# IbrahimSquared/visibility-heuristic-path-planner

Measured on AMD Instinct MI355X. Metric: visibility fields/sec on 1000x1000 grid, higher is better.
Workload: dtype f64

## Files before the change

visibility-heuristic-path-planner_amd/csrc/vhp_diag.h:

```cpp
#pragma once

#ifdef VHP_DIAG_NOSTORE
#define VHP_DIAG_STORE_GUARD(a, b, off) { asm volatile("" :: "v"(a), "v"(b), "v"(off)); return; }
#define VHP_DIAG_FRONT_STORE_GUARD if (nx != 0x7fffffff) return;
#else
#define VHP_DIAG_STORE_GUARD(a, b, off)
#define VHP_DIAG_FRONT_STORE_GUARD
#endif

#ifdef VHP_DIAG_NOXSTORE
#define VHP_DIAG_NOXSTORE_RETURN return;
#else
#define VHP_DIAG_NOXSTORE_RETURN
#endif
#ifdef VHP_DIAG_NOYSTORE
#define VHP_DIAG_NOYSTORE_RETURN return;
#define VHP_DIAG_NOYSTORE_GUARD if (m.nx == 0x7fffffff)
#else
#define VHP_DIAG_NOYSTORE_RETURN
#define VHP_DIAG_NOYSTORE_GUARD
#endif

#ifdef VHP_DIAG_PLAINSTORE
#define VHP_FIELD_STORE_PLAIN 1
#endif

#ifdef VHP_DIAG_NOWAIT
#define VHP_DIAG_NOWAIT_RETURN return;
#define VHP_DIAG_WAITS false
#else
#define VHP_DIAG_NOWAIT_RETURN
#define VHP_DIAG_WAITS true
#endif

#ifdef VHP_DIAG_NOMATH
#define VHP_DIAG_NOMATH_RETURN(x) return (x);
#else
#define VHP_DIAG_NOMATH_RETURN(x)
#endif

#if defined(VHP_DIAG_TIMELINE) && !defined(VHP_SIM)
#define VHP_DIAG_TL_DECLARE                                                                                                     \
  constexpr int kPpBins = 256;                                                                                                  \
  static __device__ unsigned long long g_pp_hist[256 * 2 * kPpBins];                                                            \
  static __device__ unsigned long long g_pp_t0;                                                                                 \
  static __device__ unsigned g_pp_unit[16384 * 2];    \
  static __device__ __forceinline__ unsigned long long* pp_slot(int which) {                                                    \
    const unsigned long long b_ = (wall_clock64() - g_pp_t0) / 1000;                                                            \
    return g_pp_hist + ((size_t)(blockIdx.x & 255) * 2 + which) * kPpBins + (b_ < kPpBins - 1 ? b_ : kPpBins - 1);              \
  }
#define VHP_DIAG_TL_ADD(which, n) do { if ((threadIdx.x & 63) == 0) atomicAdd(pp_slot(which), (unsigned long long)(long long)(n)); } while (0)
#define VHP_DIAG_TL_STRIPS(d) VHP_DIAG_TL_ADD(1, d);
#define VHP_DIAG_TL_UNIT(unit, which) do { if ((threadIdx.x & 63) == 0 && (unit) < 16384) g_pp_unit[2 * (unit) + (which)] = (unsigned)(wall_clock64() - g_pp_t0); } while (0);
#define VHP_DIAG_TL_XBLOCK(lo, hi, rows_here, j0, cb) { long c_ = 0; for (int i_ = (lo); i_ <= (hi); ++i_) c_ += ((rows_here) < i_ - (j0) + 1 ? (rows_here) : i_ - (j0) + 1); VHP_DIAG_TL_ADD(0, c_ * (cb)); }
#define VHP_DIAG_TL_YBLOCK(lo, hi, i0, ycols, ni, cb) { long c_ = 0; for (int j_ = (lo); j_ <= (hi); ++j_) { int t_ = (i0) + (ycols) - 1; if ((ni) - 1 < t_) t_ = (ni) - 1; if (j_ < t_) t_ = j_; t_ -= ((i0) > 0 ? (i0) : 0) - 1; if (t_ > 0) c_ += t_; } VHP_DIAG_TL_ADD(0, c_ * (cb)); }
#define VHP_DIAG_TL_RESET for (int k_ = threadIdx.x; k_ < 256 * 2 * kPpBins; k_ += blockDim.x) g_pp_hist[k_] = 0; if (threadIdx.x == 0) g_pp_t0 = wall_clock64();
#else
#define VHP_DIAG_TL_DECLARE
#define VHP_DIAG_TL_STRIPS(d)
#define VHP_DIAG_TL_UNIT(unit, which)
#define VHP_DIAG_TL_XBLOCK(lo, hi, rows_here, j0, cb)
#define VHP_DIAG_TL_YBLOCK(lo, hi, i0, ycols, ni, cb)
#define VHP_DIAG_TL_RESET
#endif

#ifndef VHP_PRIO_DIAG
#define VHP_PRIO_DIAG 1
#endif
#ifndef VHP_PRIO_TASK
#define VHP_PRIO_TASK 2
#endif
#if !defined(VHP_SIM) && defined(VHP_PRIO_MARCH)
#define VHP_EXP_PRIO_SET_LEFT(is_diag, left) wave_priority((is_diag) ? 3 : (left) >= VHP_PRIO_MARCH ? 2 : (left) >= VHP_PRIO_MARCH / 2 ? 1 : 0);
#define VHP_EXP_PRIO_SET(is_diag) wave_priority((is_diag) ? 3 : 0);
#define VHP_EXP_PRIO_TASK_BEGIN wave_priority(3);
#define VHP_EXP_PRIO_END wave_priority(0);
#elif !defined(VHP_SIM) && (VHP_PRIO_DIAG != 0 || VHP_PRIO_TASK != 0)
#define VHP_EXP_PRIO_SET_LEFT(is_diag, left) wave_priority((is_diag) ? VHP_PRIO_DIAG : 0);
#define VHP_EXP_PRIO_SET(is_diag) wave_priority((is_diag) ? VHP_PRIO_DIAG : 0);
#define VHP_EXP_PRIO_TASK_BEGIN wave_priority(VHP_PRIO_TASK);
#define VHP_EXP_PRIO_END wave_priority(0);
#else
#define VHP_EXP_PRIO_SET_LEFT(is_diag, left)
#define VHP_EXP_PRIO_SET(is_diag)
#define VHP_EXP_PRIO_TASK_BEGIN
#define VHP_EXP_PRIO_END
#endif

#ifndef VHP_BACKOFF_SLEEP
#define VHP_BACKOFF_SLEEP 12
#endif
#ifndef VHP_READY_SLEEP
#define VHP_READY_SLEEP 4
#endif
```

visibility-heuristic-path-planner_amd/csrc/vhp_pool.hip:

```cpp
#include "vhp_batch_launch.h"

#include <hip/hip_runtime.h>

#include "vhp.h"
#include "vhp_pool.hpp"
#include "vhp_pool_scratch.hpp"

namespace vhp {
namespace pool {

__device__ __forceinline__ void write_stamp(stamps::Entry* p, unsigned long long tag) {
  *reinterpret_cast<ulonglong2*>(p) = make_ulonglong2((unsigned long long)wall_clock64(), tag);
}

template <typename OutT, bool ANYW>
__global__ void __launch_bounds__(64 * kWaves, 1) vhp_pool_sweep(Args<OutT> a, int n_ctx, stamps::Entry* __restrict__ stamp_end) {
  extern __shared__ double lds[];
  constexpr int W = ANYW ? kWavesAny : kWaves;
  const Layout L = make_layout(W, n_ctx, a.m.nx, a.m.ny, ANYW ? kTStrideAny : kTStride);
  Worker<OutT, ANYW>::clear(lds, L, (int)threadIdx.x, 64 * W);
  __syncthreads();
  Worker<OutT, ANYW> wk;
  wk.init(a, lds, L, uniform((int)(threadIdx.x >> 6)), (int)blockIdx.x);
  wk.run();
  if (stamp_end) {
    asm volatile("s_waitcnt vmcnt(0)" ::: "memory");
    __syncthreads();
    if (threadIdx.x == 0) write_stamp(stamp_end + blockIdx.x, a.epoch);
  }
}

constexpr int kOrderLdsUnits = 8192;

template <typename Arr>
__device__ __forceinline__ int block_exclusive_scan_1024(Arr arr, int n, int* wave_tot) {
  const int per = (n + 1023) / 1024;
  const int lo = (int)threadIdx.x * per, hi = lo + per < n ? lo + per : n;
  int mine = 0;
  for (int k = lo; k < hi; ++k) mine += arr[k];
  const int lane = threadIdx.x & 63, wv = threadIdx.x >> 6;
  int inc = mine;
#pragma unroll
  for (int off = 1; off < 64; off <<= 1) {
    const int t = __shfl_up(inc, off, 64);
    if (lane >= off) inc += t;
  }
  if (lane == 63) wave_tot[wv] = inc;
  __syncthreads();
  int before = 0, all = 0;
#pragma unroll
  for (int k = 0; k < 16; ++k) { before += k < wv ? wave_tot[k] : 0; all += wave_tot[k]; }
  int at = before + inc - mine;
  for (int k = lo; k < hi; ++k) { const int v = arr[k]; arr[k] = at; at += v; }
  __syncthreads();
  return all;
}

template <typename PerUnit>
__device__ __forceinline__ void order_units(const int32_t* __restrict__ src_xy, int n_src, int nx, int ny, int* __restrict__ order,
                                            int* __restrict__ line_base, int* __restrict__ recs, long long capacity_blocks,
                                            unsigned long long* __restrict__ queue, unsigned long long queue0,
                                            int* __restrict__ err_flag, int* hist, int* wave_tot, PerUnit blocks) {
  const int n_units = n_src * kUnits;
  const double inv_area = 1.0 / ((double)nx * (double)ny), inv_side = 1.0 / (double)(nx > ny ? nx : ny);
  hist[threadIdx.x] = 0;
  __syncthreads();
  for (int u = threadIdx.x; u < n_units; u += 1024) {
    const int s = u / kUnits, qo = u - s * kUnits;
    const int sx = src_xy[2 * s], sy = src_xy[2 * s + 1];
    int nb = 0, bucket = kBuckets - 1;
    if (!(sx < 0 || sy < 0 || sx >= nx || sy >= ny)) {
      UnitGeo g;
      g.init(nx, ny, qo, sx, sy);
      nb = g.line_blocks();
      bucket = unit_launch_bucket(g, inv_area, inv_side);
    }
    blocks[u] = nb | (bucket << 20);
    atomicAdd(&hist[bucket], 1);
  }
  __syncthreads();
  (void)block_exclusive_scan_1024(hist, kBuckets, wave_tot);
  for (int u = threadIdx.x; u < n_units; u += 1024) order[atomicAdd(&hist[blocks[u] >> 20], 1)] = u;
  __syncthreads();
  for (int u = threadIdx.x; u < n_units; u += 1024) blocks[u] &= (1 << 20) - 1;
  __syncthreads();
  const int total = block_exclusive_scan_1024(blocks, n_units, wave_tot);
  const bool fits = (long long)total <= capacity_blocks;
  for (int k = threadIdx.x; k < n_units; k += 1024) {
    const int u = order[k], s = u / kUnits;
    const int sx = src_xy[2 * s], sy = src_xy[2 * s + 1];
    const bool inside = !(sx < 0 || sy < 0 || sx >= nx || sy >= ny);
    reinterpret_cast<int4*>(recs)[k] = make_int4(u, !fits ? -2 : inside ? (sx | (sy << 16)) : -1, blocks[u], 0);
  }
  if (threadIdx.x == 0) {
    *queue = fits ? queue0 : (unsigned long long)n_units;
    if (!fits) atomicOr(err_flag, 4);
  }
}

__device__ __forceinline__ void order_units_lds(const int32_t* __restrict__ src_xy, int n_src, int nx, int ny, int* __restrict__ recs,
                                                long long capacity_blocks, unsigned long long* __restrict__ queue, unsigned long long queue0,
                                                int* __restrict__ err_flag, int* hist, int* wave_tot, int* unit_key, int* src_key) {
  const int n_units = n_src * kUnits;
  const int per = (n_units + 1023) / 1024;
  const int lo = (int)threadIdx.x * per, hi = lo + per < n_units ? lo + per : n_units;
  const double inv_area = 1.0 / ((double)nx * (double)ny), inv_side = 1.0 / (double)(nx > ny ? nx : ny);
  hist[threadIdx.x] = 0;
  __syncthreads();
  int mine = 0;
  for (int u = lo; u < hi; ++u) {
    const int s = u / kUnits, qo = u - s * kUnits;
    const int sx = src_xy[2 * s], sy = src_xy[2 * s + 1];
    const bool inside = !(sx < 0 || sy < 0 || sx >= nx || sy >= ny);
    int nb = 0, bucket = kBuckets - 1;
    if (inside) {
      UnitGeo g;
      g.init(nx, ny, qo, sx, sy);
      nb = g.line_blocks();
      bucket = unit_launch_bucket(g, inv_area, inv_side);
    }
    unit_key[u] = nb | (bucket << 20);
    if (qo == 0) src_key[s] = inside ? (sx | (sy << 16)) : -1;
    mine += nb;
    atomicAdd(&hist[bucket], 1);
  }
  __syncthreads();
  const int lane = threadIdx.x & 63, wv = threadIdx.x >> 6;
  const int count = hist[threadIdx.x];
  int inc_h = count, inc_b = mine;
#pragma unroll
  for (int off = 1; off < 64; off <<= 1) {
    const int th = __shfl_up(inc_h, off, 64), tb = __shfl_up(inc_b, off, 64);
    if (lane >= off) { inc_h += th; inc_b += tb; }
  }
  if (lane == 63) { wave_tot[wv] = inc_h; wave_tot[16 + wv] = inc_b; }
  __syncthreads();
  int before_h = 0, before_b = 0, total = 0;
#pragma unroll
  for (int k = 0; k < 16; ++k) {
    before_h += k < wv ? wave_tot[k] : 0;
    before_b += k < wv ? wave_tot[16 + k] : 0;
    total += wave_tot[16 + k];
  }
  hist[threadIdx.x] = before_h + inc_h - count;
  __syncthreads();
  const bool fits = (long long)total <= capacity_blocks;
  int at = before_b + inc_b - mine;
  for (int u = lo; u < hi; ++u) {
    const int key = unit_key[u], nb = key & ((1 << 20) - 1);
    const int k = atomicAdd(&hist[key >> 20], 1);
    reinterpret_cast<int4*>(recs)[k] = make_int4(u, !fits ? -2 : src_key[u / kUnits], at, 0);
    at += nb;
  }
  if (threadIdx.x == 0) {
    *queue = fits ? queue0 : (unsigned long long)n_units;
    if (!fits) atomicOr(err_flag, 4);
  }
}

__global__ void __launch_bounds__(1024) vhp_pool_order(const int32_t* __restrict__ src_xy, int n_src, int nx, int ny, int* __restrict__ order,
                                                       int* __restrict__ line_base, int* __restrict__ recs, long long capacity_blocks,
                                                       unsigned long long* __restrict__ queue, unsigned long long queue0,
                                                       int* __restrict__ err_flag, stamps::Entry* __restrict__ stamp_begin,
                                                       unsigned long long stamp_tag) {
  if (stamp_begin && threadIdx.x == 0) write_stamp(stamp_begin, stamp_tag);
  __shared__ int hist[kBuckets];
  __shared__ int wave_tot[32];
  __shared__ int blocks[kOrderLdsUnits];
  __shared__ int src_key[kOrderLdsUnits / kUnits];
  VHP_DIAG_TL_RESET
  if (n_src * kUnits <= kOrderLdsUnits) order_units_lds(src_xy, n_src, nx, ny, recs, capacity_blocks, queue, queue0, err_flag, hist, wave_tot, blocks, src_key);
  else order_units(src_xy, n_src, nx, ny, order, line_base, recs, capacity_blocks, queue, queue0, err_flag, hist, wave_tot, line_base);
}

}

namespace {
template <typename OutT>
hipError_t launch_pool_t(const BatchArgs& a) {
  using namespace pool;
  const bool anyw = pool_needs_anyw<OutT>(a.nx, a.field_stride > 0 ? a.field_stride : (long long)a.nx * a.ny, static_cast<const OutT*>(a.d_out));
  auto k = anyw ? vhp_pool_sweep<OutT, true> : vhp_pool_sweep<OutT, false>;
  const PoolPlan p = plan_pool(a.nx, a.ny, a.n_src, a.n_cus, anyw, a.pool);
  if (!p.ok || a.pool_epoch == 0) return hipErrorInvalidValue;
  if (a.raise_lds) {
    hipError_t e = a.raise_lds(reinterpret_cast<const void*>(k), p.lds_bytes);
    if (e != hipSuccess) return e;
  }
  char* scratch = reinterpret_cast<char*>(a.d_queue);
  Args<OutT> g;
  g.m = geom_map(a);
  g.out = static_cast<OutT*>(a.d_out);
  g.field_stride = a.field_stride;
  g.err_flag = a.d_err;
  g.queue = reinterpret_cast<unsigned long long*>(a.d_queue);
  g.n_units = a.n_src * kUnits;
  int* recs = a.d_queue + kQueueInts;
  int* order = recs + 4 * (size_t)g.n_units;
  int* line_base = order + g.n_units;
  g.recs = recs;
  g.diag = reinterpret_cast<double*>(scratch + head_bytes(a.n_src));
  g.diag_stride = diag_stride_of(a.nx, a.ny);
  g.lines = reinterpret_cast<vhp::lanes::Tagged*>(scratch + head_bytes(a.n_src) + diag_bytes(a.n_src, a.nx, a.ny));
  g.epoch = a.pool_epoch;
  g.busy_cap = p.busy_cap;
  g.n_head = p.n_head;
  g.tail_limit = p.tail_limit;
  g.early_ctx = p.early_ctx;
  g.late_after = p.late_after;
  g.claim_ahead = p.claim_ahead;
  g.n_groups = a.n_cus;
  g.static_snake = p.static_snake;
  g.static_round = p.static_round;
  stamps::Entry* const stamp_end = a.d_stamps ? a.d_stamps + pool_stamp_counts(a.n_cus).n_begin : nullptr;
  if (a.ev_begin) (void)hipEventRecord(a.ev_begin, a.stream);
  hipLaunchKernelGGL(vhp_pool_order, dim3(1), dim3(1024), 0, a.stream, a.d_src, a.n_src, a.nx, a.ny, order, line_base, recs,
                     line_blocks_per_source(a.nx, a.ny) * a.n_src, reinterpret_cast<unsigned long long*>(a.d_queue), p.queue0, a.d_err,
                     a.d_stamps, a.pool_epoch);
  hipLaunchKernelGGL(k, dim3((unsigned)a.n_cus), dim3(64 * p.waves), p.lds_bytes, a.stream, g, p.n_ctx, stamp_end);
  const hipError_t e = hipGetLastError();
  if (a.ev_end) (void)hipEventRecord(a.ev_end, a.stream);
  return e;
}
}

size_t pool_scratch_bytes(int n_src, int nx, int ny) {
  return head_bytes(n_src) + diag_bytes(n_src, nx, ny) + (size_t)line_blocks_per_source(nx, ny) * (size_t)n_src * 64 * sizeof(vhp::lanes::Tagged);
}

#ifdef VHP_DIAG_TIMELINE
extern "C" int vhp_debug_read_hist(unsigned long long* dst, int n_words) {
  return (int)hipMemcpyFromSymbol(dst, HIP_SYMBOL(pool::g_pp_hist), (size_t)n_words * 8);
}
extern "C" int vhp_debug_read_units(unsigned* dst, int n_words) {
  return (int)hipMemcpyFromSymbol(dst, HIP_SYMBOL(pool::g_pp_unit), (size_t)n_words * 4);
}
#endif

hipError_t launch_pool(const BatchArgs& a) {
  if (!pool_supported(a.nx, a.ny)) return hipErrorInvalidValue;
  return a.dtype == VHP_F64 ? launch_pool_t<double>(a) : launch_pool_t<float>(a);
}

}
```

visibility-heuristic-path-planner_amd/csrc/vhp_pool.hpp:

```cpp
#pragma once
#include "vhp_geom.hpp"

namespace vhp {
namespace pool {

using namespace vhp::lanes;
using geom::imax;
using geom::imin;
using geom::Map;
using geom::Quad;

constexpr int kBlock = geom::kBlock;
constexpr int kXRows = geom::kXRows;
constexpr int kYCols = geom::kYCols;
constexpr int kLW16 = 16;
constexpr int kTStride = 17;
constexpr int kTStrideAny = 25;
constexpr int kUnits = 8;
VHP_DIAG_TL_DECLARE

constexpr int kSchedHead = 8 + 16, kCtxHead = 8;
constexpr int kHdr = 8;
constexpr int kBin = 72;
constexpr int kRing = 256;
// ... 905 lines not shown
        const vi mp = DX > 0 ? lane : 63 - lane;
        const vb end = (mp < head) || (mp >= tail);
        g_store2_mask(!end, row - 2, xoff + (uint32_t)(3 * CB), hi, nb);
        g_store2_if(end && oknb, end && !oknb, vb(false), row - 2, xoff + (uint32_t)(3 * CB), hi, nb);
      } else
        g_store2_if(okhi && oknb, okhi, oknb, row - 2, xoff + (uint32_t)(3 * CB), hi, nb);
      g_store1_if((lane == (DX > 0 ? 0 : 63)) && oklo, row, xoff, lo);
      return;
    }
    if (PRED) g_store2_if(oklo && okhi, oklo, okhi, row, xoff, lo, hi);
    else if (ANYW && VHP_POOL_SPLIT_ENDS) {
      const uint32_t k = (static_cast<uint32_t>(reinterpret_cast<uintptr_t>(row)) + static_cast<uint32_t>(piece_lo * CB)) & 63u;
      if (k == 0) { g_store2(row, xoff, lo, hi); return; }
      const int head = (int)((64u - k) / (2 * CB)), tail = 64 - (int)(k / (2 * CB));
      const vi ml = DX > 0 ? lane : 63 - lane;
      const vb end = (ml < head) || (ml >= tail);
      g_store2_mask(!end, row, xoff, lo, hi);
      g_store2_if(end, vb(false), vb(false), row, xoff, lo, hi);
    }
    else g_store2(row, xoff, lo, hi);
  }
  VHP_FN bool row_aligned(const OutT* row) const { return (reinterpret_cast<uintptr_t>(row) & (2 * CB - 1)) == 0; }
  VHP_FN OutT* row_ptr(int y) const { return out + (size_t)y * (size_t)m.nx; }

  VHP_FN void step1(int j) {
    const int y = g.Y(j);
    const int t = y & 63;
    const double rj = slab[t];
    const double dj = (double)j;
    double fill = 0.0;
    if (q > 0) fill = bin[1 + (y & 63) - DY];
    const vd b0 = shift_up(prev1, vd(fill));
    vd v0 = and_mask(stencil(prev0, b0, ratio(id0, dj, rj)), bit_mask(ow0, t));
    vd v1 = and_mask(stencil(prev1, prev0, ratio(id1, dj, rj)), bit_mask(ow1, t));
    if (j <= i0 + kYCols - 1) {
      v0 = select(ia == j, dg0, v0);
      v1 = select(ib == j, dg1, v1);
    }
    store_row<true>(row_ptr(y), j, v0, v1);
    prev0 = v0;
    prev1 = v1;
    if (has_consumer) lds_store_if(lane == 63, lk.ring, vi(y & (kRing - 1)), v1);
  }

  template <bool DIAG, bool PRED>
  VHP_FN void window8(int j0w) {
    const int y0 = g.Y(j0w);
    const int t0 = y0 & 63;
    const int yb = y0 & ~7;
    vd rr[8];
#pragma unroll
    for (int k = 0; k < 8; ++k) rr[k] = lds_bcast(slab, (yb & 63) + (DY > 0 ? k : 7 - k));
    vd rb[8];
#pragma unroll
    for (int k = 0; k < 8; ++k) rb[k] = vd(0.0);
    if (q > 0) {
      rb[0] = lds_bcast(bin, 1 + (y0 & 63) - DY);
      const int yq = 1 + (yb & 63);
#pragma unroll
      for (int k = 1; k < 8; ++k) rb[k] = lds_bcast(bin, yq + (DY > 0 ? k - 1 : 8 - k));
    }
    const int sh = DY > 0 ? (t0 & 31) : (t0 & 31) - 7;
    const vu32 hs0 = half_shifted(ow0, t0, sh), hs1 = half_shifted(ow1, t0, sh);
    double* wbase = has_consumer ? lk.ring + (yb & (kRing - 1)) : dummy;
    const vi widx = select(lane == 63, vi(0), vi((int)(dummy - wbase)));
    vd dj = vd((double)j0w);
    OutT* row = row_ptr(y0);
    const long rowstep = (long)DY * m.nx;
#pragma unroll
    for (int k = 0; k < 8; ++k) {
      const int bit = DY > 0 ? k : 7 - k;
      const vd b0 = shift_up(prev1, rb[k]);
      vd v0 = and_mask(stencil(prev0, b0, ratio(id0, dj, rr[k])), sbfe1(hs0, bit));
      vd v1 = and_mask(stencil(prev1, prev0, ratio(id1, dj, rr[k])), sbfe1(hs1, bit));
      if (DIAG) {
        v0 = select(ia == j0w + k, dg0, v0);
        v1 = select(ib == j0w + k, dg1, v1);
      }
      store_row<PRED>(row, j0w + k, v0, v1);
      prev0 = v0;
      prev1 = v1;
      lds_store(wbase, widx + bit, v1);
      dj = dj + 1.0;
      row += rowstep;
    }
  }

  VHP_FN void sweep_block(int nb) {
    int lo, hi;
    g.ysteps(nb, lo, hi);
    lo = imax(lo, jstart);
    if (lo > hi) return;
    VHP_EXP_PRIO_SET(lo <= i0 + kYCols - 1)
    const int blk = g.Y(lo) >> 6;
    {
      const vi xa = vmin(vmax(ia, 0), g.ni - 1) * DX + g.sx;
      const vi xb = vmin(vmax(ib, 0), g.ni - 1) * DX + g.sx;
      ow0 = g_load_u64(m.cols, xa * m.wpc + (1 + blk));
      ow1 = g_load_u64(m.cols, xb * m.wpc + (1 + blk));
      const vi jt = (lane + (blk * 64 - g.sy)) * DY;
      const vb ok = (jt >= 0) && (jt < g.nj);
      vd rv = select(ok, g_load_f64(m.recip, select(ok, jt, vi(0))), vd(0.0));
      pin(ow0);
      pin(ow1);
      pin(rv);
      lds_store(slab, lane, rv);
      wave_sync();
    }
    int j = lo;
    while (j <= hi) {
      const int y = g.Y(j);
      const bool aligned = DY > 0 ? (y & 7) == 0 : (y & 7) == 7;
      if (aligned && j + 7 <= hi) {
        if (q > 0) lk.fetch(j, j + 7, nb);
        if (j <= i0 + kYCols - 1) window8<true, true>(j);
        else if (!interior) window8<false, true>(j);
        else window8<false, false>(j);
        j += 8;
      } else {
        if (q > 0) lk.fetch(j, j, nb);
        step1(j);
        j += 1;
      }
      if (has_consumer) lk.publish(j);
    }
    if (has_consumer) lk.store_block(nb, blk);
    VHP_DIAG_TL_YBLOCK(lo, hi, i0, kYCols, g.ni, CB)
  }
};

template <int DX, int DY, typename OutT>
struct YStrip16 {
  static constexpr int CB = sizeof(OutT);
  static constexpr int kW = 16;
  static constexpr int kNever = 0x7fffffff;
  Map m;
  Quad<DX, DY> g;
  OutT* out;
  double* slab;
  double* bin;
  double* dummy;
  Link<DY> lk;
  int q, i0, j_first, j_last;
  bool below, has_consumer, interior;
  int blk, pf_blk, staged_blk;
  bool pf_wait;
  int tl_lo;
  vi lane, ia, ib;
  vi f0, f1;
  vd prev0, prev1, id0, id1, dg0, dg1;
  vu64 ow0, ow1, ow0_nx, ow1_nx;
  vd rv_nx;
  vu32 xoff;

  VHP_FN void init(const Map& m_, int sx, int sy, OutT* out_, const Shared& sh, int w, int q_, const double* diag) {
    m = m_; out = out_;
    g.init(m.nx, m.ny, sx, sy);
    slab = sh.lds + sh.L.slabs + w * (2 * kBlock);
    bin = lk.bin;
    dummy = sh.lds + sh.L.dummies + w * 8;
    lane = lane_id();
    q = q_;
    i0 = g.ycol0(q);
    j_first = g.ystart(q);
    j_last = g.nj - 1;
    below = q > 0;
    has_consumer = q + 1 < g.Py;
    interior = i0 >= 0 && i0 + kYCols - 1 < g.ni;
    ia = lane * 2 + i0;
    ib = ia + 1;
    prev0 = vd(0.0);
    prev1 = vd(0.0);
    id0 = to_f64(ia);
    id1 = to_f64(ib);
    const vb real0 = (ia >= 0) && (ia < g.ni), real1 = (ib >= 0) && (ib < g.ni);
    const vb zero1 = (DX < 0) ? ((ib == g.ni) && real0) : vb(false);
    f0 = select(real0, ia, vi(kNever));
    f1 = select(real1, ib, select(zero1, ia, vi(kNever)));
    dg0 = g_load_f64(diag, vmin(vmax(ia, 0), g.rows_total - 1));
    dg1 = g_load_f64(diag, vmin(vmax(ib, 0), g.rows_total - 1));
    pin(dg0);
    pin(dg1);
    dg1 = select(zero1, vd(0.0), dg1);
    const vi xlo = DX > 0 ? ia + g.sx : (-ib) + g.sx;
    xoff = to_u32(xlo * CB);
    pf_blk = -1;
    pf_wait = false;
    staged_blk = -0x7fffffff;
    blk = -0x7fffffff;
    tl_lo = j_first;
  }

  VHP_FN void load_ops(int b, vu64& o0, vu64& o1, vd& rv) {
    const vi xa = vmin(vmax(ia, 0), g.ni - 1) * DX + g.sx;
    const vi xb = vmin(vmax(ib, 0), g.ni - 1) * DX + g.sx;
    o0 = g_load_u64(m.cols, xa * m.wpc + (1 + b));
    o1 = g_load_u64(m.cols, xb * m.wpc + (1 + b));
    if (DX < 0) o1 = select(ib == g.ni, vu64(0), o1);
    const vi jt = (lane + (b * 64 - g.sy)) * DY;
    const vb ok = (jt >= 0) && (jt < g.nj);
    rv = select(ok, g_load_f64(m.recip, select(ok, jt, vi(0))), vd(0.0));
  }
  VHP_FN bool block_in_march(int b) const { const int ye = g.Y(j_last); return DY > 0 ? 64 * b <= ye : 64 * b + 63 >= ye; }
  VHP_FN void prefetch_ops(int b) { pf_blk = b; pf_wait = true; load_ops(b, ow0_nx, ow1_nx, rv_nx); }
  VHP_FN void stage(int b, vd rv) {
    wave_sync();
    lds_store(slab, lane + kBlock * (b & 1), rv);
    wave_sync();
    staged_blk = b;
  }
  VHP_FN void settle() {
    if (pf_wait) { pin(ow0_nx); pin(ow1_nx); pin(rv_nx); pf_wait = false; }
  }
  VHP_FN void stage_next() {
    if (pf_blk != -1 && staged_blk != pf_blk) { settle(); stage(pf_blk, rv_nx); }
  }
  VHP_FN void enter_block(int b) {
    if (pf_blk == b) { stage_next(); ow0 = ow0_nx; ow1 = ow1_nx; }
    else { vd rv; load_ops(b, ow0, ow1, rv); pin(ow0); pin(ow1); pin(rv); stage(b, rv); }
    blk = b;
    if (block_in_march(b + DY)) prefetch_ops(b + DY); else pf_blk = -1;
  }

  template <bool DIAG, bool PRED>
  VHP_FN void window(int ja, int yw, int nb) {
    const int k_hi = imin(kW - 1, j_last - ja);
    vd rr[kW];
#pragma unroll
    for (int k = 0; k < kW; ++k) rr[k] = lds_bcast(slab, (yw & (2 * kBlock - 1)) + (DY > 0 ? k : kW - 1 - k));
    Below16<DY> bl;
    if (below) bl.get(lk, bin, yw, DY > 0 ? yw : yw + kW - 1, imax(ja, j_first), ja + k_hi - 1, nb);
    const vu32 hs0 = half_shifted(ow0, yw & 63, yw & 31), hs1 = half_shifted(ow1, yw & 63, yw & 31);
    double* wbase = has_consumer ? lk.ring + (yw & (kRing - 1)) : dummy;
    const vi widx = select(lane == 63, vi(0), vi((int)(dummy - wbase)));
    vd dj = vd((double)ja);
    OutT* row = out + (long)g.Y(ja) * (long)m.nx;
    const long rowstep = (long)DY * m.nx;
#pragma unroll
    for (int k = 0; k < kW; ++k) {
      const int c = DY > 0 ? k : kW - 1 - k;
      const vd b0 = shift_up(prev1, below ? bl.v[k] : vd(0.0));
      vd v0 = and_mask(stencil(prev0, b0, ratio(id0, dj, rr[k])), sbfe1(hs0, c));
      vd v1 = and_mask(stencil(prev1, prev0, ratio(id1, dj, rr[k])), sbfe1(hs1, c));
      if (DIAG) {
        v0 = select(ia == ja + k, dg0, v0);
        v1 = select(ib == ja + k, dg1, v1);
      }
      VHP_DIAG_NOYSTORE_GUARD
      {
        const vd lo = DX > 0 ? v0 : v1, hi = DX > 0 ? v1 : v0;
        if (PRED) {
          const int j = ja + k <= j_last ? ja + k : -1;
          const vb ok0 = f0 <= j, ok1 = f1 <= j;
          const vb oklo = DX > 0 ? ok0 : ok1, okhi = DX > 0 ? ok1 : ok0;
          g_store2_if(oklo && okhi, oklo, okhi, row, xoff, lo, hi);
        } else {
          g_store2(row, xoff, lo, hi);
        }
      }
      prev0 = v0;
      prev1 = v1;
      lds_store(wbase, widx + c, v1);
      dj = dj + 1.0;
      row += rowstep;
    }
    if (has_consumer) lk.publish(ja + k_hi + 1);
  }

  VHP_FN void open_block(int yw, int ja) {
    const int b = yw >> 6;
    if (b == blk) return;
    if (has_consumer) lk.store_block(g.nby(ja - 1), blk);
    VHP_DIAG_TL_YBLOCK(tl_lo, ja - 1, i0, kYCols, g.ni, CB)
    tl_lo = ja;
    VHP_EXP_PRIO_SET_LEFT(ja <= i0 + kYCols - 1, j_last - ja)
    enter_block(b);
  }
  VHP_FN void run() {
    int yw = g.Y(j_first) & ~(kW - 1);
    int ja = DY > 0 ? yw - g.sy : g.sy - (yw + kW - 1);
    VHP_EXP_PRIO_SET(true)
    enter_block(yw >> 6);
    while (ja <= j_last) {
      open_block(yw, ja);
      const int nb = DY > 0 ? blk - g.by0 : g.by0 - blk;
      if (ja <= i0 + kYCols - 1) window<true, true>(ja, yw, nb);
      else if (!interior || ja + kW - 1 > j_last) window<false, true>(ja, yw, nb);
      else window<false, false>(ja, yw, nb);
      ja += kW; yw += kW * DY;
      sim_progress();
      sim_point();
    }
    if (has_consumer) lk.store_block(imax(g.nby(imin(imax(ja - 1, 0), j_last)), 0), blk);
    VHP_DIAG_TL_YBLOCK(tl_lo, j_last, i0, kYCols, g.ni, CB)
  }
};

template <int DX, int DY>
struct DiagTask {
  Map m;
  Quad<DX, DY> g;
  double* diag;
  int k;
  vi lane;
  vd dprev, sprev;

  VHP_FN void init(const Map& m_, int sx, int sy, double* diag_) {
    m = m_;
    g.init(m.nx, m.ny, sx, sy);
    diag = diag_;
    lane = lane_id();
    k = 0;
    dprev = vd(0.0);
    sprev = vd(0.0);
  }
  VHP_FN bool done() const { return k >= g.rows_total; }
  VHP_FN int run_chunk() {
    const int k0 = k, k1 = imin(k0 + kBlock, g.rows_total);
    const vi kk = vmin(lane + k0, g.rows_total - 1);
    const vi x = kk * DX + g.sx;
    const vi ya = vmax(kk - 1, 0) * DY + g.sy, yb = kk * DY + g.sy;
    const vu64 wa = g_load_u64(m.rows, ya * m.wpr + ((x >> 6) + 1));
    const vu64 wb = g_load_u64(m.rows, yb * m.wpr + ((x >> 6) + 1));
    const vd rk = g_load_f64(m.recip, kk);
    const vi ma = bit_mask_lane(wa, x & 63), mb = bit_mask_lane(wb, x & 63);
    const vd cv = ratio(to_f64(vmax(kk - 1, 0)), to_f64(kk), rk);
    vd acc = vd(0.0);
    for (int kq = k0; kq < k1; ++kq) {
      const int l = kq - k0;
      vd dcur;
      if (kq == 0) {
        dcur = and_mask(vd(1.0), vi(read_lane_i(mb, l)));
        sprev = vd(0.0);
      } else {
        const vd c = vd(read_lane(cv, l));
        const vd sub = and_mask(stencil(dprev, sprev, c), vi(read_lane_i(ma, l)));
        dcur = and_mask(sub, vi(read_lane_i(mb, l)));
        sprev = sub;
      }
      dprev = dcur;
      acc = select(lane == l, dcur, acc);
    }
    g_store_f64_if(lane < (k1 - k0), diag, lane + k0, acc);
    k = k1;
    return k1;
  }
};

enum { kFound = 0, kRetry = 1, kIdle = 2, kExit = 3 };


template <typename OutT>
VHP_HD bool pool_needs_anyw(int nx, long long field_stride, const OutT* out) {
  return (nx & 7) != 0 || (field_stride & 1) != 0 || (reinterpret_cast<uintptr_t>(out) & (2 * sizeof(OutT) - 1)) != 0;
}

#ifndef VHP_POOL_X8
#define VHP_POOL_X16 1
#else
#define VHP_POOL_X16 0
#endif

template <typename OutT, bool ANYW = false>
struct Worker {
  static constexpr bool kUseX16 = !ANYW && VHP_POOL_X16 != 0;
#ifdef VHP_POOL_Y8
  static constexpr bool kUseY16 = false, kMayY16 = false;
#else
  static constexpr bool kUseY16 = kUseX16;
#ifdef VHP_POOL_ANYW_Y16
  static constexpr bool kMayY16 = ANYW && VHP_POOL_X16 != 0;
#else
  static constexpr bool kMayY16 = false;
#endif
#endif
  Args<OutT> a;
  Shared sh;
  int w, group;
  bool pairs_aligned;
  vi lane;

  VHP_FN void init(const Args<OutT>& a_, double* lds, const Layout& L, int w_, int group_) {
    a = a_;
    pairs_aligned = (a_.m.nx & 1) == 0 && (a_.field_stride & 1) == 0 && (reinterpret_cast<uintptr_t>(a_.out) & (2 * sizeof(OutT) - 1)) == 0;
    sh.lds = lds;
    sh.L = L;
    w = w_;
    group = group_;
    lane = lane_id();
  }

  static VHP_FN void clear(double* lds, const Layout& L, int tid, int nthreads) {
    Shared s;
    s.lds = lds;
    s.L = L;
    int* sc = s.sched();
    const int n = kSchedHead + L.C * L.ctx_stride;
    for (int k = tid; k < n; k += nthreads) lds_set_int(sc + k, 0);
  }

  VHP_FN int find_work(int& c_out, int& p_out, int& qo_out, int& sx_out, int& sy_out) {
    int* sc = sh.sched();
    int best_c = -1, best_seq = 0x7fffffff, best_p = 0, best_word = 0, best_qo = 0, best_sx = 0, best_sy = 0;
    int free_c = -1, free_first = -1;
    bool unclaimed = false, installing = false;
    const bool late_open = a.early_ctx >= sh.L.C || lds_poll(sc + kLateOpen) != 0;
    const int first_done = a.static_round ? lds_poll(sc + kFirstDone) : -1;
    for (int c = 0; c < sh.L.C; ++c) {
      int* cx = sh.ctx(c);
      const int st = lds_poll(cx + kState);
      if (st == 0) {
        if (((first_done >> c) & 1) == 0) free_first = c;
        else if (c < a.early_ctx || late_open) free_c = c;
        continue;
      }
      if (st == 1) { installing = true; continue; }
      const int word = lds_poll(cx + kWord);
      if (word < 0) continue;
      const int p = word & 255, seq = word >> 8;
      const int ns = lds_poll(cx + kNStrips);
      if (p >= ns) continue;
      unclaimed = true;
      const int rank = c < a.n_head ? c : seq + 16;
      if (rank >= best_seq) continue;
      const int unit = lds_poll(cx + kUnit), sxsy = lds_poll(cx + kSxSy);
      const int qo = unit & 7, sx = sxsy & 0xffff, sy = sxsy >> 16;
      UnitGeo ug;
      ug.init(a.m.nx, a.m.ny, qo, sx, sy);
      if (VHP_DIAG_WAITS && p > 0 && lds_poll(sh.prog(c) + (p - 1)) < ug.first_step(p) + 8 + 1 - a.claim_ahead) continue;
      if (VHP_DIAG_WAITS && !ug.x_major && lds_poll(cx + kDiagReady) < ug.diag_need(p)) continue;
      best_c = c; best_seq = rank; best_p = p; best_word = word; best_qo = qo; best_sx = sx; best_sy = sy;
    }
    if (best_c >= 0) {
      sim_point();
      if (lds_cas(sh.ctx(best_c) + kWord, best_word, best_word + 1) != best_word) return kRetry;
      lds_set_int(sh.owner(best_c) + best_p, w);
      c_out = best_c; p_out = best_p; qo_out = best_qo; sx_out = best_sx; sy_out = best_sy;
      sim_progress();
      return kFound;
    }
    const bool q_empty = lds_poll(sc + kQEmpty) != 0;
    if (free_first >= 0) free_c = free_first;
    if (free_c >= 0 && (!q_empty || free_first >= 0) && lds_poll(sc + kBusy) < a.busy_cap) {
      sim_point();
      if (lds_cas(sh.ctx(free_c) + kState, 0, 1) == 0) {
        install(free_c);
      }
      return kRetry;
    }
    if (q_empty && !unclaimed && !installing && free_first < 0) return kExit;
    return kIdle;
  }

  VHP_FN void install(int c) {
    int* sc = sh.sched();
    int* cx = sh.ctx(c);
    int idx;
    if (a.static_round && ((lds_poll(sc + kFirstDone) >> c) & 1) == 0) {
      lds_or(sc + kFirstDone, 1 << c);
      const int slot = (a.static_snake && (c & 1)) ? a.n_groups - 1 - group : group;
      idx = c < a.n_head ? c * a.n_groups + slot : a.n_units - 1 - ((c - a.n_head) * a.n_groups + group);
      sim_progress();
    } else {
      bool from_tail = c >= a.n_head;
      if (from_tail && (int)(g_peek_u64(a.queue) >> 32) >= a.tail_limit) from_tail = false;
      const unsigned long long old = g_add_u64(a.queue, from_tail ? (1ull << 32) : 1ull);
      const unsigned taken_head = (unsigned)old, taken_tail = (unsigned)(old >> 32);
      idx = from_tail ? a.n_units - 1 - (int)taken_tail : (int)taken_head;
      if ((int)(taken_head + taken_tail) >= a.late_after) lds_publish(sc + kLateOpen, 1);
      sim_progress();
      if (taken_head + taken_tail >= (unsigned)a.n_units) {
        lds_publish(sc + kQEmpty, 1);
        lds_publish(cx + kState, 0);
        return;
      }
    }
    int unit, sxsy, lbase, rsvd;
    g_load_rec4(a.recs, idx, unit, sxsy, lbase, rsvd);
    const int s = unit / kUnits, qo = unit - s * kUnits;
    if (sxsy < 0) {
      if (qo == 0 && sxsy == -1) g_store_scalar_if(lane == 0, a.err_flag, vi(0), 1);
      lds_publish(cx + kState, 0);
      return;
    }
    const int sx = sxsy & 0xffff, sy = sxsy >> 16;
    VHP_DIAG_TL_UNIT(unit, 0)
    UnitGeo ug;
    ug.init(a.m.nx, a.m.ny, qo, sx, sy);
    OutT* field = a.out + (size_t)s * a.field_stride;
    if (qo == 0) {
      if (sy > 0)
        for (int x0 = 0; x0 < a.m.nx; x0 += kLanes) g_store_scalar_if(lane + x0 < a.m.nx, field, lane + x0, OutT(0));
    }
    if (ug.n_strips == 0) {
      lds_publish(cx + kState, 0);
      return;
    }
    lds_set_int(cx + kUnit, unit);
    lds_set_int(cx + kNStrips, ug.n_strips);
    lds_set_int(cx + kLeft, ug.n_strips);
    lds_set_int(cx + kSxSy, sxsy);
    lds_set_int(cx + kDiagReady, 0);
    lds_set_int(cx + kLineBase, lbase);
    for (int k0 = 0; k0 < ug.n_strips; k0 += kLanes) lds_store_i_if(lane + k0 < ug.n_strips, sh.prog(c), lane + k0, 0);
    const int seq = lds_add(sc + kSeq, 1) + 1;
    lds_publish(cx + kWord, seq << 8);
    lds_publish(cx + kState, 2);
    if (!ug.x_major) {
      double* dline = a.diag + (size_t)(4 * s + (qo >> 1)) * a.diag_stride;
      switch (qo >> 1) {
        case 0: run_diag<+1, +1>(cx, sx, sy, dline); break;
        case 1: run_diag<-1, +1>(cx, sx, sy, dline); break;
        case 2: run_diag<-1, -1>(cx, sx, sy, dline); break;
        default: run_diag<+1, -1>(cx, sx, sy, dline); break;
      }
    }
  }

  template <int DX, int DY>
  VHP_FN void run_diag(int* cx, int sx, int sy, double* dline) {
    DiagTask<DX, DY> dt;
    dt.init(a.m, sx, sy, dline);
    VHP_EXP_PRIO_TASK_BEGIN
    while (!dt.done()) {
      const int ready = dt.run_chunk();
      stores_done();
      lds_publish(cx + kDiagReady, ready);
      sim_progress();
      sim_point();
    }
    VHP_EXP_PRIO_END
  }

  VHP_FN void strip_done(int c) {
    int* cx = sh.ctx(c);
    if (lds_add(cx + kLeft, -1) == 1) {
      VHP_DIAG_TL_UNIT(lds_int_at(cx + kUnit), 1)
      lds_publish(cx + kWord, -1);
      lds_publish(cx + kState, 0);
    }
    sim_progress();
  }

  VHP_FN Tagged* line_of(int c, int p, int nb) const { return a.lines + (size_t)64 * ((size_t)lds_int_at(sh.ctx(c) + kLineBase) + (size_t)p * nb); }
  VHP_FN int tag_of(int c, int p) const { return (((lds_int_at(sh.ctx(c) + kWord) >> 8) & 0x1ff) << 8) | p; }

  template <int DX, int DY>
  VHP_FN void run_x(int c, int unit, int p, int sx, int sy, OutT* field) {
    Quad<DX, DY> g;
    g.init(a.m.nx, a.m.ny, sx, sy);
    int* mine = sh.prog(c) + p;
    if (kUseX16) {
      XStrip16<DX, DY, OutT> xs;
      xs.lk.init(sh, w, sx, kXRows * p, tag_of(c, p), mine, p > 0 ? line_of(c, p - 1, g.Nbx) : nullptr, p + 1 < g.Px ? line_of(c, p, g.Nbx) : nullptr,
                 a.epoch, p > 0 ? lds_int_at(sh.owner(c) + (p - 1)) : -1, p > 0 ? tag_of(c, p - 1) : 0);
      xs.init(a.m, sx, sy, field, sh, w, p);
      VHP_DIAG_TL_STRIPS(1)
      xs.run();
    } else {
      XStrip<DX, DY, OutT, ANYW> xs;
      xs.lk.init(sh, w, sx, kXRows * p, tag_of(c, p), mine, p > 0 ? line_of(c, p - 1, g.Nbx) : nullptr, p + 1 < g.Px ? line_of(c, p, g.Nbx) : nullptr,
                 a.epoch, p > 0 ? lds_int_at(sh.owner(c) + (p - 1)) : -1, p > 0 ? tag_of(c, p - 1) : 0);
      xs.init(a.m, sx, sy, field, sh, w, p);
      VHP_DIAG_TL_STRIPS(1)
      for (int n = p; n < xs.g.Nbx; ++n) {
        xs.sweep_block(n);
        if (n == xs.g.Nbx - 1) xs.end_of_march();
        sim_progress();
        sim_point();
      }
    }
    lds_publish(mine, 0x3fff);
    VHP_DIAG_TL_STRIPS(-1)
    strip_done(c);
  }

  template <int DX, int DY>
  VHP_FN void run_y(int c, int unit, int q, int sx, int sy, OutT* field, const double* dline) {
    Quad<DX, DY> g;
    g.init(a.m.nx, a.m.ny, sx, sy);
    int* mine = sh.prog(c) + q;
    if (kUseY16 || (kMayY16 && pairs_aligned)) {
      YStrip16<DX, DY, OutT> ys;
      ys.lk.init(sh, w, sy, g.ystart(q), tag_of(c, q), mine, q > 0 ? line_of(c, q - 1, g.Nby) : nullptr, q + 1 < g.Py ? line_of(c, q, g.Nby) : nullptr,
                 a.epoch, q > 0 ? lds_int_at(sh.owner(c) + (q - 1)) : -1, q > 0 ? tag_of(c, q - 1) : 0);
      ys.init(a.m, sx, sy, field, sh, w, q, dline);
      VHP_DIAG_TL_STRIPS(1)
      ys.run();
    } else {
      YStrip<DX, DY, OutT, ANYW> ys;
      ys.lk.init(sh, w, sy, g.ystart(q), tag_of(c, q), mine, q > 0 ? line_of(c, q - 1, g.Nby) : nullptr, q + 1 < g.Py ? line_of(c, q, g.Nby) : nullptr,
                 a.epoch, q > 0 ? lds_int_at(sh.owner(c) + (q - 1)) : -1, q > 0 ? tag_of(c, q - 1) : 0);
      ys.init(a.m, sx, sy, field, sh, w, q, dline);
      VHP_DIAG_TL_STRIPS(1)
      for (int n = ys.g.nby(ys.jstart); n < ys.g.Nby; ++n) {
        ys.sweep_block(n);
        sim_progress();
        sim_point();
      }
    }
    lds_publish(mine, 0x3fff);
    VHP_DIAG_TL_STRIPS(-1)
    strip_done(c);
  }

  VHP_FN void run_strip(int c, int p, int qo, int sx, int sy) {
    const int unit = lds_int_at(sh.ctx(c) + kUnit);
    const int s = unit / kUnits;
    OutT* field = a.out + (size_t)s * a.field_stride;
    const double* dline = a.diag + (size_t)(4 * s + (qo >> 1)) * a.diag_stride;
    switch (qo) {
      case 0: run_x<+1, +1>(c, unit, p, sx, sy, field); break;
      case 1: run_y<+1, +1>(c, unit, p, sx, sy, field, dline); break;
      case 2: run_x<-1, +1>(c, unit, p, sx, sy, field); break;
      case 3: run_y<-1, +1>(c, unit, p, sx, sy, field, dline); break;
      case 4: run_x<-1, -1>(c, unit, p, sx, sy, field); break;
      case 5: run_y<-1, -1>(c, unit, p, sx, sy, field, dline); break;
      case 6: run_x<+1, -1>(c, unit, p, sx, sy, field); break;
      default: run_y<+1, -1>(c, unit, p, sx, sy, field, dline); break;
    }
  }

  VHP_FN void run() {
    for (;;) {
      int c = 0, p = 0, qo = 0, sx = 0, sy = 0;
      const int r = find_work(c, p, qo, sx, sy);
      if (r == kExit) break;
      if (r == kIdle) { backoff(); continue; }
      if (r == kRetry) continue;
      lds_add(sh.sched() + kBusy, 1);
      run_strip(c, p, qo, sx, sy);
      VHP_EXP_PRIO_END
      lds_add(sh.sched() + kBusy, -1);
    }
  }
};

}
}
```

Before: 447,700.

## Limit diagonal precompute to rows consumed by y-strips and add hold-time probes

The diagonal task now stops after the number of entries the y-strips actually consume (kYCols*Py - ya) rather than all rows_total, which drops diagonal work that no strip reads. The diff also adds timeline diagnostics that measure how long y-major strips wait on diagonal readiness, plus per-unit start and diag-done stamps. These diagnostics compile to nothing unless VHP_DIAG_TIMELINE is defined. The risk is a mismatch in the entry count if some consumer needs rows beyond that bound.

```diff
diff --git a/visibility-heuristic-path-planner_amd/csrc/vhp_diag.h b/visibility-heuristic-path-planner_amd/csrc/vhp_diag.h
--- a/visibility-heuristic-path-planner_amd/csrc/vhp_diag.h
+++ b/visibility-heuristic-path-planner_amd/csrc/vhp_diag.h
@@ -44,23 +44,38 @@
   constexpr int kPpBins = 256;                                                                                                  \
   static __device__ unsigned long long g_pp_hist[256 * 2 * kPpBins];                                                            \
   static __device__ unsigned long long g_pp_t0;                                                                                 \
-  static __device__ unsigned g_pp_unit[16384 * 2];    \
+   \
+  static __device__ unsigned g_pp_unit[16384 * 4];                                                                              \
+   \
+  static __device__ unsigned long long g_pp_held[256 * 4];                                                                      \
+  static __device__ unsigned long long g_pp_since[256 * 16];    \
   static __device__ __forceinline__ unsigned long long* pp_slot(int which) {                                                    \
     const unsigned long long b_ = (wall_clock64() - g_pp_t0) / 1000;                                                            \
     return g_pp_hist + ((size_t)(blockIdx.x & 255) * 2 + which) * kPpBins + (b_ < kPpBins - 1 ? b_ : kPpBins - 1);              \
+  }                                                                                                                             \
+  static __device__ __forceinline__ void pp_held(unsigned long long since) {                                                    \
+    if ((threadIdx.x & 63) != 0 || since == 0) return;                                                                          \
+    atomicAdd(g_pp_held + (blockIdx.x & 255) * 4 + 1, 1ull);                                                                    \
+    atomicAdd(g_pp_held + (blockIdx.x & 255) * 4 + 2, wall_clock64() - since);                                                  \
   }
 #define VHP_DIAG_TL_ADD(which, n) do { if ((threadIdx.x & 63) == 0) atomicAdd(pp_slot(which), (unsigned long long)(long long)(n)); } while (0)
 #define VHP_DIAG_TL_STRIPS(d) VHP_DIAG_TL_ADD(1, d);
-#define VHP_DIAG_TL_UNIT(unit, which) do { if ((threadIdx.x & 63) == 0 && (unit) < 16384) g_pp_unit[2 * (unit) + (which)] = (unsigned)(wall_clock64() - g_pp_t0); } while (0);
+#define VHP_DIAG_TL_UNIT(unit, which) do { if ((threadIdx.x & 63) == 0 && (unit) < 16384) g_pp_unit[4 * (unit) + (which)] = (unsigned)(wall_clock64() - g_pp_t0); } while (0);
 #define VHP_DIAG_TL_XBLOCK(lo, hi, rows_here, j0, cb) { long c_ = 0; for (int i_ = (lo); i_ <= (hi); ++i_) c_ += ((rows_here) < i_ - (j0) + 1 ? (rows_here) : i_ - (j0) + 1); VHP_DIAG_TL_ADD(0, c_ * (cb)); }
 #define VHP_DIAG_TL_YBLOCK(lo, hi, i0, ycols, ni, cb) { long c_ = 0; for (int j_ = (lo); j_ <= (hi); ++j_) { int t_ = (i0) + (ycols) - 1; if ((ni) - 1 < t_) t_ = (ni) - 1; if (j_ < t_) t_ = j_; t_ -= ((i0) > 0 ? (i0) : 0) - 1; if (t_ > 0) c_ += t_; } VHP_DIAG_TL_ADD(0, c_ * (cb)); }
-#define VHP_DIAG_TL_RESET for (int k_ = threadIdx.x; k_ < 256 * 2 * kPpBins; k_ += blockDim.x) g_pp_hist[k_] = 0; if (threadIdx.x == 0) g_pp_t0 = wall_clock64();
+#define VHP_DIAG_TL_HELD_MARK(c) do { unsigned long long* s_ = g_pp_since + (blockIdx.x & 255) * 16 + ((c) & 15); if ((threadIdx.x & 63) == 0 && *s_ == 0) *s_ = wall_clock64(); } while (0);
+#define VHP_DIAG_TL_HELD_CLAIM(c, y_major) do { unsigned long long* s_ = g_pp_since + (blockIdx.x & 255) * 16 + ((c) & 15); if (y_major) pp_held(*s_); if ((threadIdx.x & 63) == 0) *s_ = 0; } while (0);
+#define VHP_DIAG_TL_YSTRIP if ((threadIdx.x & 63) == 0) atomicAdd(g_pp_held + (blockIdx.x & 255) * 4, 1ull);
+#define VHP_DIAG_TL_RESET for (int k_ = threadIdx.x; k_ < 256 * 2 * kPpBins; k_ += blockDim.x) g_pp_hist[k_] = 0; for (int k_ = threadIdx.x; k_ < 256 * 4; k_ += blockDim.x) g_pp_held[k_] = 0; for (int k_ = threadIdx.x; k_ < 256 * 16; k_ += blockDim.x) g_pp_since[k_] = 0; if (threadIdx.x == 0) g_pp_t0 = wall_clock64();
 #else
 #define VHP_DIAG_TL_DECLARE
 #define VHP_DIAG_TL_STRIPS(d)
 #define VHP_DIAG_TL_UNIT(unit, which)
 #define VHP_DIAG_TL_XBLOCK(lo, hi, rows_here, j0, cb)
 #define VHP_DIAG_TL_YBLOCK(lo, hi, i0, ycols, ni, cb)
+#define VHP_DIAG_TL_HELD_MARK(c)
+#define VHP_DIAG_TL_HELD_CLAIM(c, y_major)
+#define VHP_DIAG_TL_YSTRIP
 #define VHP_DIAG_TL_RESET
 #endif
 
diff --git a/visibility-heuristic-path-planner_amd/csrc/vhp_pool.hip b/visibility-heuristic-path-planner_amd/csrc/vhp_pool.hip
--- a/visibility-heuristic-path-planner_amd/csrc/vhp_pool.hip
+++ b/visibility-heuristic-path-planner_amd/csrc/vhp_pool.hip
@@ -235,6 +235,9 @@
 extern "C" int vhp_debug_read_units(unsigned* dst, int n_words) {
   return (int)hipMemcpyFromSymbol(dst, HIP_SYMBOL(pool::g_pp_unit), (size_t)n_words * 4);
 }
+extern "C" int vhp_debug_read_held(unsigned long long* dst, int n_words) {
+  return (int)hipMemcpyFromSymbol(dst, HIP_SYMBOL(pool::g_pp_held), (size_t)n_words * 8);
+}
 #endif
 
 hipError_t launch_pool(const BatchArgs& a) {
diff --git a/visibility-heuristic-path-planner_amd/csrc/vhp_pool.hpp b/visibility-heuristic-path-planner_amd/csrc/vhp_pool.hpp
--- a/visibility-heuristic-path-planner_amd/csrc/vhp_pool.hpp
+++ b/visibility-heuristic-path-planner_amd/csrc/vhp_pool.hpp
@@ -1231,6 +1231,7 @@
   Quad<DX, DY> g;
   double* diag;
   int k;
+  int n_entries;
   vi lane;
   vd dprev, sprev;
 
@@ -1240,12 +1241,13 @@
     diag = diag_;
     lane = lane_id();
     k = 0;
+    n_entries = imin(kYCols * g.Py - g.ya, g.rows_total);
     dprev = vd(0.0);
     sprev = vd(0.0);
   }
-  VHP_FN bool done() const { return k >= g.rows_total; }
+  VHP_FN bool done() const { return k >= n_entries; }
   VHP_FN int run_chunk() {
-    const int k0 = k, k1 = imin(k0 + kBlock, g.rows_total);
+    const int k0 = k, k1 = imin(k0 + kBlock, n_entries);
     const vi kk = vmin(lane + k0, g.rows_total - 1);
     const vi x = kk * DX + g.sx;
     const vi ya = vmax(kk - 1, 0) * DY + g.sy, yb = kk * DY + g.sy;
@@ -1357,13 +1359,14 @@
       UnitGeo ug;
       ug.init(a.m.nx, a.m.ny, qo, sx, sy);
       if (VHP_DIAG_WAITS && p > 0 && lds_poll(sh.prog(c) + (p - 1)) < ug.first_step(p) + 8 + 1 - a.claim_ahead) continue;
-      if (VHP_DIAG_WAITS && !ug.x_major && lds_poll(cx + kDiagReady) < ug.diag_need(p)) continue;
+      if (VHP_DIAG_WAITS && !ug.x_major && lds_poll(cx + kDiagReady) < ug.diag_need(p)) { VHP_DIAG_TL_HELD_MARK(c) continue; }
       best_c = c; best_seq = rank; best_p = p; best_word = word; best_qo = qo; best_sx = sx; best_sy = sy;
     }
     if (best_c >= 0) {
       sim_point();
       if (lds_cas(sh.ctx(best_c) + kWord, best_word, best_word + 1) != best_word) return kRetry;
       lds_set_int(sh.owner(best_c) + best_p, w);
+      VHP_DIAG_TL_HELD_CLAIM(best_c, (best_qo & 1) != 0)
       c_out = best_c; p_out = best_p; qo_out = best_qo; sx_out = best_sx; sy_out = best_sy;
       sim_progress();
       return kFound;
@@ -1459,6 +1462,7 @@
       sim_point();
     }
     VHP_EXP_PRIO_END
+    VHP_DIAG_TL_UNIT(lds_int_at(cx + kUnit), 3)
   }
 
   VHP_FN void strip_done(int c) {
@@ -1485,6 +1489,7 @@
                  a.epoch, p > 0 ? lds_int_at(sh.owner(c) + (p - 1)) : -1, p > 0 ? tag_of(c, p - 1) : 0);
       xs.init(a.m, sx, sy, field, sh, w, p);
       VHP_DIAG_TL_STRIPS(1)
+      if (p == 0) { VHP_DIAG_TL_UNIT(unit, 2) }
       xs.run();
     } else {
       XStrip<DX, DY, OutT, ANYW> xs;
@@ -1492,6 +1497,7 @@
                  a.epoch, p > 0 ? lds_int_at(sh.owner(c) + (p - 1)) : -1, p > 0 ? tag_of(c, p - 1) : 0);
       xs.init(a.m, sx, sy, field, sh, w, p);
       VHP_DIAG_TL_STRIPS(1)
+      if (p == 0) { VHP_DIAG_TL_UNIT(unit, 2) }
       for (int n = p; n < xs.g.Nbx; ++n) {
         xs.sweep_block(n);
         if (n == xs.g.Nbx - 1) xs.end_of_march();
@@ -1515,6 +1521,8 @@
                  a.epoch, q > 0 ? lds_int_at(sh.owner(c) + (q - 1)) : -1, q > 0 ? tag_of(c, q - 1) : 0);
       ys.init(a.m, sx, sy, field, sh, w, q, dline);
       VHP_DIAG_TL_STRIPS(1)
+      VHP_DIAG_TL_YSTRIP
+      if (q == 0) { VHP_DIAG_TL_UNIT(unit, 2) }
       ys.run();
     } else {
       YStrip<DX, DY, OutT, ANYW> ys;
@@ -1522,6 +1530,8 @@
                  a.epoch, q > 0 ? lds_int_at(sh.owner(c) + (q - 1)) : -1, q > 0 ? tag_of(c, q - 1) : 0);
       ys.init(a.m, sx, sy, field, sh, w, q, dline);
       VHP_DIAG_TL_STRIPS(1)
+      VHP_DIAG_TL_YSTRIP
+      if (q == 0) { VHP_DIAG_TL_UNIT(unit, 2) }
       for (int n = ys.g.nby(ys.jstart); n < ys.g.Nby; ++n) {
         ys.sweep_block(n);
         sim_progress();
```

Result: no change. 447,500 (-0.0%).
